# 001cat/pySurfInv

Hardware: AMD Instinct MI355X
Metric: layered-model dispersion forward solves/sec (20 periods) (higher is better)
Workload: dtype f32 (root search, Love group velocity) + f64 (Rayleigh eigenfunction state)

## Files before the change

pysurfinv_amd/csrc/surfdisp_kernels.hip:

```cpp
#include <hip/hip_runtime.h>
#include <stdint.h>
#include <type_traits>
#include <atomic>
#include "surfdisp_internal.h"

#define SD_HD __host__ __device__
#ifndef SD_CERT_STRIDE
#define SD_CERT_STRIDE 6
#endif

namespace sd {

constexpr float R0      = 6371.0f;
constexpr float PI_REF  = 3.1415927f;
constexpr float DC      = 0.01f;
constexpr float FACT    = 4.0f;
constexpr float ACCUR   = 1.e-8f;
constexpr float CLUSTER_DC = 1.0e-4f;

enum { F_VP = 0, F_VS, F_RHO, F_QS, F_DIF, F_QQQ, F_DFL, F_HSF, F_HSR, NF = 9 };

SD_HD __forceinline__ bool fin(float x) { return fabsf(x) <= 3.402823466e38f; }
SD_HD __forceinline__ float pwr_of(int kind) { return kind == 1 ? 5.0f : 2.2750f; }

// ... 1493 lines not shown
    const int mmf = (hk >> 16) & 0x3fff;
    const size_t fs = (size_t)A.Lmax * B;
    const float c = A.c[idx], T = A.per[k];
    struct Replay { int kk, nflat; float lnT; };
    const Replay r0{k, hk & 0xffff, logf(1.0f / T)};
    auto layer = [&](int i, Replay &r) -> LayerV {
        while (r.nflat <= i && r.kk > 0) {
            --r.kk;
            const int h = A.hist[(size_t)r.kk * B + b];
            r.nflat = (h < 0) ? n : (h & 0xffff);
            r.lnT = logf(1.0f / A.per[r.kk]);
        }
        return layer_derive(layer_load(A.mdl, fs, (size_t)i * B + b), r.lnT, i == r.nflat - 1);
    };
    const int last = mmf - 1;
    float v2 = 0.0f, v3 = 0.0f;
    bool exact = A.only_flagged != 0;
    if (!exact) {
        const RTrial t = ray_trial(c, T);
        int kk = k;
        int nflat = hk & 0xffff;
        float lnT = r0.lnT;
        RState s2{}, s3{};
        float phi = 0.0f, rho_prev = 0.0f;
        RLyr y{};
        float rho_i = 0.0f;
        for (int i = 0; i <= last; ++i) {
            while (nflat <= i && kk > 0) {
                --kk;
                const int h = A.hist[(size_t)kk * B + b];
                nflat = (h < 0) ? n : (h & 0xffff);
                lnT = logf(1.0f / A.per[kk]);
            }
            const LayerV v = layer_derive(layer_load(A.mdl, fs, (size_t)i * B + b), lnT, i == nflat - 1);
            rho_prev = rho_i;
            rho_i = v.rho;
            y.sv = v.b; y.d = v.d;
            y.ia2 = wk_ia2(v.a);
            y.ib2 = wk_ib2(v.b);
            y.rat = (i > 0) ? wk_rat(rho_prev, rho_i) : 0.0f;
            if (i == 0) {
                const float irho0 = wk_irho(rho_i);
                s2 = ray_start(t, 2, irho0);
                s3 = ray_start(t, 3, irho0);
                if (last >= 1) { ray_step<true>(s2, t, y, 2, phi); ray_step<true>(s3, t, y, 3, phi); }
            } else if (i < last) {
                ray_step<false>(s2, t, y, 2, phi);
                ray_step<false>(s3, t, y, 3, phi);
            }
        }
        const float rp = (last >= 1) ? rho_prev : 0.0f;
        float m2 = 0.0f, m3 = 0.0f;
        v2 = ray_close(s2, t, y, rho_i, rp, 2, &m2); v3 = ray_close(s3, t, y, rho_i, rp, 3, &m3);
        const float b2max = A.ovf ? 0.5f * __expf(0.25f * A.ovf[2 * (size_t)B + b]) : 0.0f;
        exact = (A.ell_ambig < 0.0f) ||
                ((A.ell_ambig > 0.0f) && (fabsf(v2) < A.ell_ambig * m2 || fabsf(v3) < A.ell_ambig * m3 || 2.0f * b2max > A.ell_gmax * c * c));
    }
    if (exact) {
        Replay r = r0;
        v2 = delta_rayleigh_ref_gen([&](int m) { const LayerV v = layer(m, r); return RefLyr{v.a, v.b, v.rho, v.d}; }, mmf, c, T, 2);
        r = r0;
        v3 = delta_rayleigh_ref_gen([&](int m) { const LayerV v = layer(m, r); return RefLyr{v.a, v.b, v.rho, v.d}; }, mmf, c, T, 3);
        if (A.amb_count) atomicAdd(A.amb_count + 1, 1);
    }
    A.ratio[idx] = 0.5f * v3 / v2;
}

struct Drop { int hs_layer; int nreg_hs; };

template <int KIND>
SD_HD __forceinline__ Drop drop_group(const float *__restrict__ mdl, size_t fs, int B, int b,
                                           int n, float lnT, float c, float T, int ndiv, bool water,
                                           float div)
{
    const float dmax = FACT * T * c;
    float sum = 0.0f;
    Drop r; r.hs_layer = n - 1; r.nreg_hs = 0;
    LayerRaw nraw = layer_load(mdl, fs, (size_t)b);
    for (int jl = 0; jl < n; ++jl) {
        const LayerRaw raw = nraw;
        if (jl + 1 < n) nraw = layer_load(mdl, fs, (size_t)(jl + 1) * B + b);
        const LayerV v = layer_derive(raw, lnT, jl == n - 1);
        if (!(c < v.b)) continue;
        if (jl == n - 1) break;
        const int nsub = (jl == 0 && water) ? 1 : ndiv;
        const float dsub = (ndiv > 1 && !(jl == 0 && water)) ? v.d / div : v.d;
        for (int s = 0; s < nsub; ++s) sum = sum + dsub;
        if (!(sum > dmax)) continue;
        const LayerV nx = layer_derive(nraw, lnT, jl + 1 == n - 1);
        bool lower, equal;
        if (KIND == 2) {
            lower = (nx.a < v.a) || (nx.a == v.a && nx.b < v.b);
            equal = (nx.a == v.a) && (nx.b == v.b);
        } else {
            lower = nx.b < v.b;
            equal = nx.b == v.b;
        }
        if (lower) { r.hs_layer = jl; r.nreg_hs = nsub - 1; break; }
        if (equal) continue;
        r.hs_layer = jl + 1; r.nreg_hs = 0; break;
    }
    return r;
}

struct KOut {
    float *b;
    size_t stride;
    ptrdiff_t off_a, off_r;
    int raw;
    SD_HD void put(int i, float vb, float va, float vr) const
    {
        float *q = b + (size_t)i * stride;
        *q = vb;
        if (off_a) *reinterpret_cast<float *>(reinterpret_cast<char *>(q) + off_a) = va;
        if (off_r) *reinterpret_cast<float *>(reinterpret_cast<char *>(q) + off_r) = vr;
    }
};
struct K3 { float b, a, r; };
struct Chain { float dbdb, dadb, dada, rfac; };
SD_HD __forceinline__ Chain chain_of(const LayerRaw &r, float lnT, bool is_halfspace, bool raw)
{
    if (raw) return Chain{1.0f, 0.0f, 1.0f, 1.0f};
    const float qsq = r.qs * lnT / PI_REF;
    const float qpq = qsq * 1.33333333f * (r.b_ref * r.b_ref) / (r.a_ref * r.a_ref);
    const float vfac = is_halfspace ? r.hsf : r.dif;
    Chain ch;
    ch.dbdb = (1.0f + qsq) * vfac;
    ch.dadb = 2.66666667f * qsq * (r.b_ref / r.a_ref) * vfac;
    ch.dada = (1.0f - qpq) * vfac;
    ch.rfac = is_halfspace ? r.hsr : r.qqq;
    return ch;
}
struct KC { float b1, b2, a, r; };
SD_HD __forceinline__ KC kern_coef(const LayerRaw &raw, const LayerV &v, float lnT, bool is_halfspace, float cw, bool rawc)
{
    const Chain ch = chain_of(raw, lnT, is_halfspace, rawc);
    const float rc2 = 2.0f * v.rho * cw;
    return KC{rc2 * v.b * ch.dbdb, rc2 * v.a * ch.dadb, rc2 * v.a * ch.dada, cw * ch.rfac / v.rho};
}
#ifndef SD_KERN_REAL
#define SD_KERN_REAL double
#endif
typedef SD_KERN_REAL KR;
SD_HD __forceinline__ K3 kern_layer_rayleigh(const KC &kc, float rho, float xlamb, float xmu, float wvno, float wvnosq,
                                             float omegsq, KR dmmr, KR dmmz, KR drsz, KR dzsr, KR smmz, KR smmr)
{
    const KR two = 2, k2 = wvnosq, tk = 2.0f * wvno;
    const KR dldl = -k2 * dmmr + tk * drsz - smmz;
    const KR dldm = -k2 * (two * dmmr + dmmz) - tk * dzsr - (two * smmz + smmr);
    const KR dldr = (KR)omegsq * (dmmr + dmmz);
    return K3{(float)((KR)kc.b1 * (dldm - two * dldl) + (KR)kc.b2 * dldl), (float)((KR)kc.a * dldl),
              (float)((KR)kc.r * ((KR)rho * dldr + (KR)xlamb * dldl + (KR)xmu * dldm))};
}

struct RCoef { float a12, a13, a21, a24, a31, a34, a42, a43, ddz; };

struct RInt {
    double i0, i1, i2;
};

struct M2x2 { double a, b, c, d; };
SD_HD __forceinline__ M2x2 mm(const M2x2 &x, const M2x2 &y)
{
#pragma clang fp contract(off)
    M2x2 r;
    r.a = fma(x.a, y.a, x.b * y.c); r.b = fma(x.a, y.b, x.b * y.d);
    r.c = fma(x.c, y.a, x.d * y.c); r.d = fma(x.c, y.b, x.d * y.d);
    return r;
}
SD_HD __forceinline__ M2x2 mm2(const M2x2 &x, const M2x2 &y, const M2x2 &u, const M2x2 &v)
{
#pragma clang fp contract(off)
    M2x2 r;
    r.a = fma(x.a, y.a, fma(x.b, y.c, fma(u.a, v.a, u.b * v.c))); r.b = fma(x.a, y.b, fma(x.b, y.d, fma(u.a, v.b, u.b * v.d)));
    r.c = fma(x.c, y.a, fma(x.d, y.c, fma(u.c, v.a, u.d * v.c))); r.d = fma(x.c, y.b, fma(x.d, y.d, fma(u.c, v.b, u.d * v.d)));
    return r;
}
SD_HD __forceinline__ M2x2 madd(const M2x2 &x, const M2x2 &y)
{
    M2x2 r; r.a = x.a + y.a; r.b = x.b + y.b; r.c = x.c + y.c; r.d = x.d + y.d; return r;
}
struct RProp { M2x2 p11, p12, p21, p22; };

SD_HD __forceinline__ RProp make_prop(const RCoef &q)
{
#pragma clang fp contract(off)
    const double wh = (double)(0.5f * q.ddz), w1 = (double)(1.0f * q.ddz);
    const double t6 = (double)((1.0f / 6.0f) * q.ddz), t3 = (double)((1.0f / 3.0f) * q.ddz);
    const double k1 = (t6 + t3) + (t3 + t6);
    const double k2 = (t3 * wh + t3 * wh) + t6 * w1;
    const double k3 = t3 * wh * wh + t6 * w1 * wh;
    const double k4 = t6 * w1 * wh * wh;
    const M2x2 m1 = {(double)q.a31, (double)q.a34, (double)q.a21, (double)q.a24};
    const M2x2 m2 = {(double)q.a13, (double)q.a12, (double)q.a43, (double)q.a42};
    RProp P;
    auto diag_block = [&](const M2x2 &nn) -> M2x2 {
        const double tr = nn.a + nn.d;
        const double det = fma(nn.a, nn.d, -(nn.b * nn.c));
        const double al = fma(k4, tr, k2), be = fma(-k4, det, 1.0);
        return M2x2{fma(al, nn.a, be), al * nn.b, al * nn.c, fma(al, nn.d, be)};
    };
    auto off_block = [&](const M2x2 &nn, const M2x2 &m) -> M2x2 {
        const M2x2 q = {fma(k3, nn.a, k1), k3 * nn.b, k3 * nn.c, fma(k3, nn.d, k1)};
        return mm(q, m);
    };
    {
        const M2x2 n1 = mm(m1, m2);
        P.p11 = diag_block(n1);
        P.p12 = off_block(n1, m1);
    }
    {
        const M2x2 n2 = mm(m2, m1);
        P.p22 = diag_block(n2);
        P.p21 = off_block(n2, m2);
    }
    return P;
}
struct RPow { double f0, f1, g0, g1; };
struct RBase { M2x2 m1, m2, n1, n2; double t, d; RPow p; };
SD_HD __forceinline__ RBase make_base(const RCoef &q)
{
#pragma clang fp contract(off)
    const double wh = (double)(0.5f * q.ddz), w1 = (double)(1.0f * q.ddz);
    const double t6 = (double)((1.0f / 6.0f) * q.ddz), t3 = (double)((1.0f / 3.0f) * q.ddz);
    const double k1 = (t6 + t3) + (t3 + t6);
    const double k2 = (t3 * wh + t3 * wh) + t6 * w1;
    const double k3 = t3 * wh * wh + t6 * w1 * wh;
    const double k4 = t6 * w1 * wh * wh;
    RBase r;
    r.m1 = M2x2{(double)q.a31, (double)q.a34, (double)q.a21, (double)q.a24};
    r.m2 = M2x2{(double)q.a13, (double)q.a12, (double)q.a43, (double)q.a42};
    r.n1 = mm(r.m1, r.m2);
    r.n2 = mm(r.m2, r.m1);
    r.t = r.n1.a + r.n1.d;
    r.d = fma(r.n1.a, r.n1.d, -(r.n1.b * r.n1.c));
    r.p = RPow{fma(-k4, r.d, 1.0), fma(k4, r.t, k2), k1, k3};
    return r;
}
SD_HD __forceinline__ RPow pow_mul(const RPow &x, const RPow &y, double t, double d)
{
#pragma clang fp contract(off)
    const double ff = x.f1 * y.f1, gg = x.g1 * y.g1, fg = fma(x.f1, y.g1, x.g1 * y.f1);
    const double a0 = fma(x.f0, y.f0, -d * ff), a1 = fma(x.f0, y.f1, fma(x.f1, y.f0, t * ff));
    const double b0 = fma(x.g0, y.g0, -d * gg), b1 = fma(x.g0, y.g1, fma(x.g1, y.g0, t * gg));
    RPow r;
    r.f0 = fma(-d, b1, a0);
    r.f1 = fma(t, b1, a1 + b0);
    r.g0 = fma(x.f0, y.g0, fma(x.g0, y.f0, -d * fg));
    r.g1 = fma(x.f0, y.g1, fma(x.f1, y.g0, fma(x.g0, y.f1, fma(x.g1, y.f0, t * fg))));
    return r;
}
SD_HD __forceinline__ RPow pow_sq(const RPow &x, double t, double d)
{
#pragma clang fp contract(off)
    const double ff = x.f1 * x.f1, gg = x.g1 * x.g1, fg = x.f1 * x.g1;
    const double a0 = fma(x.f0, x.f0, -d * ff), a1 = fma(2.0 * x.f0, x.f1, t * ff);
    const double b0 = fma(x.g0, x.g0, -d * gg), b1 = fma(2.0 * x.g0, x.g1, t * gg);
    RPow r;
    r.f0 = fma(-d, b1, a0);
    r.f1 = fma(t, b1, a1 + b0);
    r.g0 = 2.0 * fma(x.f0, x.g0, -d * fg);
    r.g1 = 2.0 * fma(x.f0, x.g1, fma(x.f1, x.g0, t * fg));
    return r;
}
SD_HD __forceinline__ RPow pow_sublayers(const RBase &L, int nreg)
{
    RPow q = pow_sq(pow_sq(L.p, L.t, L.d), L.t, L.d);
    RPow r = (nreg & 1) ? q : RPow{1.0, 0.0, 0.0, 0.0};
    for (int e = nreg >> 1; e > 0; e >>= 1) {
        q = pow_sq(q, L.t, L.d);
        if (e & 1) r = pow_mul(r, q, L.t, L.d);
    }
    return r;
}
SD_HD __forceinline__ RProp pow_expand(const RBase &L, const RPow &x)
{
#pragma clang fp contract(off)
    RProp P;
    P.p11 = M2x2{fma(x.f1, L.n1.a, x.f0), x.f1 * L.n1.b, x.f1 * L.n1.c, fma(x.f1, L.n1.d, x.f0)};
    P.p22 = M2x2{fma(x.f1, L.n2.a, x.f0), x.f1 * L.n2.b, x.f1 * L.n2.c, fma(x.f1, L.n2.d, x.f0)};
    P.p12 = mm(M2x2{fma(x.g1, L.n1.a, x.g0), x.g1 * L.n1.b, x.g1 * L.n1.c, fma(x.g1, L.n1.d, x.g0)}, L.m1);
    P.p21 = mm(M2x2{fma(x.g1, L.n2.a, x.g0), x.g1 * L.n2.b, x.g1 * L.n2.c, fma(x.g1, L.n2.d, x.g0)}, L.m2);
    return P;
}
SD_HD __forceinline__ RProp prop_sq(const RProp &P)
{
    RProp Q;
    Q.p11 = mm2(P.p11, P.p11, P.p12, P.p21);
    Q.p12 = mm2(P.p11, P.p12, P.p12, P.p22);
    Q.p21 = mm2(P.p21, P.p11, P.p22, P.p21);
    Q.p22 = mm2(P.p21, P.p12, P.p22, P.p22);
    return Q;
}
SD_HD __forceinline__ void prop_apply(const RProp &P, double v[4])
{
#pragma clang fp contract(off)
    const double ur = v[0], uz = v[1], tz = v[2], tr = v[3];
    v[0] = fma(P.p11.a, ur, fma(P.p11.b, tz, fma(P.p12.a, uz, P.p12.b * tr)));
    v[2] = fma(P.p11.c, ur, fma(P.p11.d, tz, fma(P.p12.c, uz, P.p12.d * tr)));
    v[1] = fma(P.p21.a, ur, fma(P.p21.b, tz, fma(P.p22.a, uz, P.p22.b * tr)));
    v[3] = fma(P.p21.c, ur, fma(P.p21.d, tz, fma(P.p22.c, uz, P.p22.d * tr)));
}

template <int MODE, bool KERN = false>
SD_HD __forceinline__ void rayleigh_sweep(const float *__restrict__ mdl, size_t fs, int B, int b,
                                               int n, float lnT, int ndiv, bool water, float div,
                                               const Drop dr, float wvno, float wvnosq, float omegsq,
                                               double y[4], double z[4], bool do_y,
                                               double xnorm, double bbn, RInt &acc,
                                               const KOut ko = KOut{nullptr, 1, 0, 0, 0}, float cw = 0.0f, K3 *hold = nullptr)
{
#pragma clang fp contract(off)
    LayerRaw nraw = layer_load(mdl, fs, (size_t)dr.hs_layer * B + b);
    for (int jl = dr.hs_layer; jl >= 0; --jl) {
        const LayerRaw raw = nraw;
        if (jl > 0) nraw = layer_load(mdl, fs, (size_t)(jl - 1) * B + b);
        const int nsub = (jl == 0 && water) ? 1 : ndiv;
        const int nreg = (jl == dr.hs_layer) ? dr.nreg_hs : nsub;
        if (nreg <= 0) continue;
        const LayerV v = layer_derive(raw, lnT, jl == n - 1);
        if (v.b <= 0.0f) {
            if (MODE == 2 && KERN && jl > 0) ko.put(jl, 0.0f, 0.0f, 0.0f);
            continue;
        }
        const float dsub = (ndiv > 1 && !(jl == 0 && water)) ? v.d / div : v.d;
        const float xmu = v.rho * v.b * v.b;
        const float xlamb = v.rho * (v.a * v.a - 2.0f * v.b * v.b);
        KC kc{};
        if (MODE == 2 && KERN) kc = kern_coef(raw, v, lnT, jl == n - 1, cw, ko.raw != 0);
        RCoef q;
        q.ddz = -dsub / (4.0f * 1.0f);
        q.a12 = 1.0f / (xlamb + 2.0f * xmu);
        q.a13 = wvno * xlamb * q.a12;
        q.a21 = -omegsq * v.rho;
        q.a24 = wvno; q.a31 = -wvno;
        q.a34 = 1.0f / xmu;
        q.a42 = -q.a13;
        q.a43 = q.a21 + 4.0f * wvnosq * xmu * (xlamb + xmu) * q.a12;
        if (MODE == 0) {
            const RBase L = make_base(q);
            const RProp Pm = pow_expand(L, pow_sublayers(L, nreg));
            if (do_y) prop_apply(Pm, y);
            prop_apply(Pm, z);
            continue;
        }
        const RProp P = make_prop(q);
        if (MODE == 1) {
            for (int s = 0; s < nreg; ++s) {
#pragma unroll
                for (int kk = 3; kk >= 0; --kk) {
                    if (do_y) prop_apply(P, y);
                    prop_apply(P, z);
                }
            }
            continue;
        }
        const bool two_vec = do_y;
        const float dz = dsub / 4.0f;
        const float l2m = xlamb + 2.0f * xmu;
        const float ixmu = q.a34, il2m = q.a12;
        float f_mr[5], f_mz[5], f_rz[5], f_zr[5];
        constexpr bool kern = KERN;
        KR k_mr = 0, k_mz = 0, k_rz = 0, k_zr = 0, k_sz = 0, k_sr = 0;
#ifdef SD_KERN_BOOLE_INCR
        float w_sz = 0.0f, w_sr = 0.0f, t_sz = 0.0f, t_sr = 0.0f;
#else
        float f_sz[5], f_sr[5];
#endif
        const double ibb = 1.0 / bbn;
        auto knot = [&](int kk) {
            float aur, auz, atz, atr;
            if (two_vec) {
                aur = (float)((xnorm * y[0] + z[0]) * ibb); auz = (float)((xnorm * y[1] + z[1]) * ibb);
                atz = (float)((xnorm * y[2] + z[2]) * ibb); atr = (float)((xnorm * y[3] + z[3]) * ibb);
            } else {
                aur = (float)z[0]; auz = (float)z[1]; atz = (float)z[2]; atr = (float)z[3];
            }
            const float durdz = atr * ixmu - wvno * auz;
            const float duzdz = (atz + wvno * xlamb * aur) * il2m;
            f_mr[kk] = aur * aur; f_mz[kk] = auz * auz;
            f_rz[kk] = aur * duzdz; f_zr[kk] = auz * durdz;
            if (kern) {
#ifdef SD_KERN_BOOLE_INCR
                t_sz = duzdz * duzdz; t_sr = durdz * durdz;
                const float wk = (kk == 2) ? 12.0f : ((kk & 1) ? 32.0f : 7.0f);
                w_sz = fmaf(wk, t_sz, w_sz); w_sr = fmaf(wk, t_sr, w_sr);
#else
                f_sz[kk] = duzdz * duzdz; f_sr[kk] = durdz * durdz;
#endif
            }
        };
        for (int s = 0; s < nreg; ++s) {
            if (s == 0) knot(4);
            else { f_mr[4] = f_mr[0]; f_mz[4] = f_mz[0]; f_rz[4] = f_rz[0]; f_zr[4] = f_zr[0];
#ifdef SD_KERN_BOOLE_INCR
                   if (kern) { w_sz = 7.0f * t_sz; w_sr = 7.0f * t_sr; }
#else
                   if (kern) { f_sz[4] = f_sz[0]; f_sr[4] = f_sr[0]; }
#endif
            }
#pragma unroll
            for (int kk = 3; kk >= 0; --kk) {
                if (two_vec) prop_apply(P, y);
                prop_apply(P, z);
                knot(kk);
            }
            const float hq = dz / 22.5f;
#define SD_BOOLE(v) (hq * (7.0f * (v[0] + v[4]) + 32.0f * (v[1] + v[3]) + 12.0f * v[2]))
            const float dmmr = SD_BOOLE(f_mr), dmmz = SD_BOOLE(f_mz);
            const float drsz = SD_BOOLE(f_rz), dzsr = SD_BOOLE(f_zr);
            if (kern) {
                k_mr += dmmr; k_mz += dmmz; k_rz += drsz; k_zr += dzsr;
#ifdef SD_KERN_BOOLE_INCR
                k_sz += hq * w_sz; k_sr += hq * w_sr;
#else
                k_sz += SD_BOOLE(f_sz); k_sr += SD_BOOLE(f_sr);
#endif
            }
#undef SD_BOOLE
            acc.i0 += (double)(v.rho * (dmmr + dmmz));
            acc.i1 += (double)(l2m * dmmr + xmu * dmmz);
            acc.i2 += (double)(xmu * dzsr - xlamb * drsz);
        }
        if (kern) {
            const K3 sh = kern_layer_rayleigh(kc, v.rho, xlamb, xmu, wvno, wvnosq, omegsq, k_mr, k_mz, k_rz, k_zr, k_sz, k_sr);
            if (jl == dr.hs_layer) *hold = sh;
            else ko.put(jl, sh.b, sh.a, sh.r);
        }
    }
}

#ifdef SD_COUNT_RESTARTS
__device__ unsigned long long sd_restart_count[2];
#endif

template <bool KERN = false>
SD_HD float group_rayleigh(const float *__restrict__ mdl, size_t fs, int B, int b, int n,
                                float T, float c, float ratio, double *dbg = nullptr,
                                const KOut ko = KOut{nullptr, 1, 0, 0, 0}, float *kscale = nullptr, int *khs = nullptr)
{
#pragma clang fp contract(off)
    const float lnT = logf(1.0f / T);
    int ndiv = 5;
    const int ivre = 99 / (n - 1);
    if (ndiv > ivre) ndiv = ivre;
    if (ndiv < 1) ndiv = 1;
    const float div = (float)ndiv;
    const LayerV top = layer_at(mdl, fs, (size_t)b, lnT, false);
    const bool water = (ndiv > 1) ? (top.b <= 0.1e-10f) : false;
    const bool wet = !(top.b > 0.0f);
    const Drop dr = drop_group<2>(mdl, fs, B, b, n, lnT, c, T, ndiv, water, div);
    const float wvno = 6.2831853072f / (c * T);
    const float wvnosq = wvno * wvno;
    const float omega = 6.2831853072f / T;
    const float omegsq = omega * omega;
    RInt acc; acc.i0 = 0.0; acc.i1 = 0.0; acc.i2 = 0.0;
    float tzz = 0.0f;
    const float cw = c / wvno;
    K3 hold{0.0f, 0.0f, 0.0f};
    if (KERN) { *kscale = 0.0f; *khs = dr.hs_layer; }
    float wat_a = 0.0f, wat_r = 0.0f;
    if (wet) {
        const float d1 = top.d;
        const float xl1 = top.rho * (top.a * top.a - 2.0f * top.b * top.b);
        const float ra = c / top.a;
        const float cr1 = ra * ra - 1.0f;
        const float mag = wvno * sqrtf(fabsf(cr1));
        if (mag <= 1.0e-35f) {
            acc.i0 = top.rho * d1;
        } else {
            float sin2ra, cosra, rab1, sinra_over;
            if (cr1 >= 0.0f) {
                sin2ra = sinf(2.0f * mag * d1) / (4.0f * mag);
                cosra = cosf(mag * d1);
                rab1 = mag * mag;
                sinra_over = sinf(mag * d1) / mag;
            } else {
                sin2ra = sinhf(2.0f * mag * d1) / (4.0f * mag);
                cosra = coshf(mag * d1);
                rab1 = -(mag * mag);
                sinra_over = sinhf(mag * d1) / mag;
            }
            const float cos2rm = 1.0f / (cosra * cosra);
            const float fac1 = (0.5f * d1 + sin2ra) * cos2rm;
            const float fac3 = wvno * (0.5f * d1 - sin2ra) * cos2rm;
            const float fac2 = wvno * fac3 / rab1;
            acc.i0 = top.rho * (fac1 + fac2);
            acc.i1 = xl1 * fac2;
            acc.i2 = xl1 * fac3;
            tzz = -top.rho * omegsq * sinra_over / cosra;
            if (KERN && !ko.raw) {
                const LayerRaw wraw = layer_load(mdl, fs, (size_t)b);
                const Chain ch = chain_of(wraw, lnT, false, false);
                const float dldl = -wvnosq * (ra * ra) * (ra * ra) * fac2;
                const float dldr = omegsq * (fac1 + fac2);
                wat_a = 2.0f * top.rho * top.a * cw * dldl * ch.dada;
                wat_r = cw * (dldr + top.a * top.a * dldl) * ch.rfac;
            }
        }
        if (KERN) ko.put(0, 0.0f, wat_a, wat_r);
    }
    const LayerV hsv = layer_at(mdl, fs, (size_t)dr.hs_layer * B + b, lnT, dr.hs_layer == n - 1);
    const float cova = c / hsv.a, covb = c / hsv.b;
    const float gam = 2.0f / (covb * covb);
    const float gamm1 = gam - 1.0f;
    const float ra = wvno * sqrtf(fabsf(cova * cova - 1.0f));
    const float rb = wvno * sqrtf(fabsf(covb * covb - 1.0f));
    const float det = wvnosq - ra * rb;
    const float h = hsv.rho * omegsq;
    const float brkt = -gamm1 * wvno + gam * ra * rb / wvno;
    const double y0[4] = {1.0, 0.0, (double)(-h * brkt / det), (double)(-h * ra / det)};
    double z0[4] = {0.0, 1.0, (double)(-h * rb / det), (double)(-h * brkt / det)};
    double y[4], z[4];
    double xnorm = 0.0, bbn = 1.0;
    auto fit = [&](auto step_tag) -> double {
        constexpr int STEP = decltype(step_tag)::value;
        for (int i = 0; i < 4; ++i) { y[i] = y0[i]; z[i] = z0[i]; }
        rayleigh_sweep<STEP>(mdl, fs, B, b, n, lnT, ndiv, water, div, dr, wvno, wvnosq, omegsq,
                             y, z, true, 0.0, 1.0, acc);
        const double yt0 = y[0], yt1 = y[1];
        double aa = z[0] - ratio * z[1];
        double bb = ratio * yt1 - yt0;
        if (fabs(bb) < 1.e-10) bb = copysign(1.e-10, bb);
        xnorm = aa / bb;
        bb = xnorm * yt1 + z[1];
        if (fabs(bb) < 1.e-10) bb = copysign(1.e-10, bb);
        bbn = bb;
        const float ampur = (float)((xnorm * yt0 + z[0]) / bb);
        const float xtest = fabsf(ampur / ratio - 1.0f);
#if defined(SD_COUNT_RESTARTS) && defined(__HIP_DEVICE_COMPILE__)
        if (STEP == 0) {
            const unsigned long long m = __ballot(xtest >= 0.00001f);
            if (m && (__lane_id() == __ffsll(__ballot(1)) - 1)) atomicAdd(&sd_restart_count[1], 1ull);
            if (xtest >= 0.00001f) atomicAdd(&sd_restart_count[0], 1ull);
        }
#endif
        if (xtest >= 0.00001f) {
            for (int i = 0; i < 4; ++i) z0[i] = z0[i] + xnorm * y0[i];
            if (STEP == 0) {
                for (int i = 0; i < 4; ++i) z[i] = z[i] + xnorm * y[i];
            } else {
                for (int i = 0; i < 4; ++i) z[i] = z0[i];
                rayleigh_sweep<STEP>(mdl, fs, B, b, n, lnT, ndiv, water, div, dr, wvno, wvnosq, omegsq,
                                     y, z, false, 0.0, 1.0, acc);
            }
            aa = z[0] - ratio * z[1];
            bb = ratio * yt1 - yt0;
            if (fabs(bb) < 1.e-10) bb = copysign(1.e-10, bb);
            xnorm = aa / bb;
            bb = xnorm * yt1 + z[1];
            if (fabs(bb) < 1.e-10) bb = copysign(1.e-10, bb);
            bbn = bb;
        }
        return fmax(fmax(fabs(yt0), fabs(yt1)), fmax(fabs(z[0]), fabs(z[1]))) / fabs(bbn);
    };
    const double z0_orig[4] = {z0[0], z0[1], z0[2], z0[3]};
    const double cancel = fit(std::integral_constant<int, 0>{});
    if (dbg) { for (int i = 0; i < 4; ++i) { dbg[i] = y[i]; dbg[4 + i] = z[i]; } dbg[12] = dr.hs_layer; dbg[13] = dr.nreg_hs; dbg[14] = ndiv; dbg[8] = xnorm; dbg[9] = bbn; }
    float aur, auz;
    const bool any_solid = (dr.hs_layer > (wet ? 1 : 0)) || (dr.nreg_hs > 0);
    (void)tzz;
    if (cancel <= 1.0e7) {
        for (int i = 0; i < 4; ++i) { z[i] = (xnorm * y0[i] + z0[i]) / bbn; y[i] = 0.0; }
        aur = (float)z[0]; auz = (float)z[1];
        rayleigh_sweep<2, KERN>(mdl, fs, B, b, n, lnT, ndiv, water, div, dr, wvno, wvnosq, omegsq,
                                y, z, false, xnorm, bbn, acc, ko, cw, &hold);
    } else {
        for (int i = 0; i < 4; ++i) z0[i] = z0_orig[i];
        (void)fit(std::integral_constant<int, 1>{});
        for (int i = 0; i < 4; ++i) { y[i] = y0[i]; z[i] = z0[i]; }
        aur = (float)((xnorm * y0[0] + z0[0]) / bbn);
        auz = (float)((xnorm * y0[1] + z0[1]) / bbn);
        rayleigh_sweep<2, KERN>(mdl, fs, B, b, n, lnT, ndiv, water, div, dr, wvno, wvnosq, omegsq,
                                y, z, true, xnorm, bbn, acc, ko, cw, &hold);
    }
    if (wet && !any_solid) { aur = ratio; auz = 1.0f; }
    {
        const float xmu = hsv.rho * hsv.b * hsv.b;
        const float xlamb = hsv.rho * (hsv.a * hsv.a - 2.0f * hsv.b * hsv.b);
        const float ap = -hsv.rho * (wvno * aur + rb * auz) / det;
        const float bp = -hsv.rho * (-ra * aur / wvno - auz) / det;
        const float a1 = -wvno * ap / hsv.rho;
        const float a2 = -wvno * rb * bp / hsv.rho;
        const float a3 = ra * ap / hsv.rho;
        const float a4 = wvnosq * bp / hsv.rho;
        if (rb == 0.0f) return hsv.b;
        const double dmmr = a1 * a1 / (2.0f * ra) + 2.0f * a1 * a2 / (ra + rb) + a2 * a2 / (2.0f * rb);
        const double dmmz = a3 * a3 / (2.0f * ra) + 2.0f * a3 * a4 / (ra + rb) + a4 * a4 / (2.0f * rb);
        const double drsz = -a1 * a3 / 2.0f - (a1 * a4 * rb + a2 * a3 * ra) / (ra + rb) - a2 * a4 / 2.0f;
        const double dzsr = -a1 * a3 / 2.0f - (a1 * a4 * ra + a2 * a3 * rb) / (ra + rb) - a2 * a4 / 2.0f;
        acc.i0 += hsv.rho * (dmmr + dmmz);
        acc.i1 += (xlamb + 2.0f * xmu) * dmmr + xmu * dmmz;
        acc.i2 += xmu * dzsr - xlamb * drsz;
        if (KERN) {
            const float smmz = ra * a3 * a3 / 2.0f + 2.0f * ra * rb * a3 * a4 / (ra + rb) + rb * a4 * a4 / 2.0f;
            const float smmr = ra * a1 * a1 / 2.0f + 2.0f * ra * rb * a1 * a2 / (ra + rb) + rb * a2 * a2 / 2.0f;
            const LayerRaw hraw = layer_load(mdl, fs, (size_t)dr.hs_layer * B + b);
            const K3 sh = kern_layer_rayleigh(kern_coef(hraw, hsv, lnT, dr.hs_layer == n - 1, cw, ko.raw != 0), hsv.rho, xlamb, xmu,
                                              wvno, wvnosq, omegsq, (KR)dmmr, (KR)dmmz, (KR)drsz, (KR)dzsr, (KR)smmz, (KR)smmr);
            ko.put(dr.hs_layer, hold.b + sh.b, hold.a + sh.a, hold.r + sh.r);
        }
    }
    if (dbg) { dbg[10] = acc.i0; dbg[11] = acc.i1; dbg[15] = acc.i2; }
    const float s0 = (float)acc.i0, s1 = (float)acc.i1, s2 = (float)acc.i2;
    if (KERN) *kscale = 1.0f / (-2.0f * (wvno * s1 + s2));
    return (wvno * s1 + s2) / (omega * s0);
}

template <bool KERN = false>
SD_HD float group_love(const float *__restrict__ mdl, size_t fs, int B, int b, int n,
                            float T, float c, const KOut ko = KOut{nullptr, 1, 0, 0, 0}, float *kscale = nullptr, int *khs = nullptr)
{
    const float lnT = logf(1.0f / T);
    int ndiv = 5;
    const int ivre = 999 / (n - 1);
    if (ndiv > ivre) ndiv = ivre;
    if (ndiv < 1) ndiv = 1;
    const float div = (float)ndiv;
    const LayerV top = layer_at(mdl, fs, (size_t)b, lnT, false);
    const bool water = (ndiv > 1) ? (top.b <= 0.1e-10f) : false;
    const Drop dr = drop_group<1>(mdl, fs, B, b, n, lnT, c, T, ndiv, water, div);
    const float wvno = 6.2831853f / (c * T);
    const LayerV hsv = layer_at(mdl, fs, (size_t)dr.hs_layer * B + b, lnT, dr.hs_layer == n - 1);
    constexpr bool kern = KERN;
    const float wvnosq = wvno * wvno;
    const float omega = 6.2831853f / T, omegsq = omega * omega;
    const float cw = c / wvno;
    auto kern_layer = [&](int jl, const LayerRaw &raw, const LayerV &v, float dm, float sm) -> K3 {
        const Chain ch = chain_of(raw, lnT, jl == n - 1, ko.raw != 0);
        const float dldm = -(wvnosq * dm + sm);
        const float dldr = omegsq * dm;
        return K3{2.0f * v.rho * v.b * cw * dldm * ch.dbdb, 0.0f, cw * (dldr + v.b * v.b * dldm) * ch.rfac};
    };
    if (kern) { *kscale = 0.0f; *khs = dr.hs_layer; }
    float ut0 = 1.0f;
    for (int attempt = 0; attempt < 16; ++attempt) {
        float ut = ut0;
        K3 hold{0.0f, 0.0f, 0.0f};
        const float covb = c / hsv.b;
        const float hh = hsv.rho * hsv.b * hsv.b;
        const float rbh = wvno * sqrtf(fabsf(covb * covb - 1.0f));
        float tq = -hh * rbh * ut0;
        const float dm0 = (rbh == 0.0f) ? 1.0e25f : 0.5f / rbh;
        float sumi0 = hsv.rho * dm0;
        float sumi1 = hh * dm0;
        bool overflow = false;
        LayerRaw nraw = layer_load(mdl, fs, (size_t)dr.hs_layer * B + b);
        if (kern && rbh > 0.0f) hold = kern_layer(dr.hs_layer, nraw, hsv, dm0, 0.5f * rbh);
        for (int jl = dr.hs_layer; jl >= 0 && !overflow; --jl) {
            const LayerRaw raw = nraw;
            if (jl > 0) nraw = layer_load(mdl, fs, (size_t)(jl - 1) * B + b);
            const int nsub = (jl == 0 && water) ? 1 : ndiv;
            const int nreg = (jl == dr.hs_layer) ? dr.nreg_hs : nsub;
            if (nreg <= 0) continue;
            const LayerV v = layer_derive(raw, lnT, jl == n - 1);
            if (v.b == 0.0f) {
                if (fabsf(ut) > 1.0e10f) overflow = true;
                if (kern && jl != dr.hs_layer) ko.put(jl, 0.0f, 0.0f, 0.0f);
                continue;
            }
            const float dsub = (ndiv > 1 && !(jl == 0 && water)) ? v.d / div : v.d;
            const float cv = c / v.b;
            const float rb = wvno * sqrtf(fabsf(cv * cv - 1.0f));
            const float h = v.rho * v.b * v.b;
            const float dz = dsub / 4.0f;
            float yk[4], zk[4], ck[4];
#pragma unroll
            for (int kk = 0; kk < 4; ++kk) {
                const float xkk = (float)(kk + 1);
                const float q = rb * dz * xkk;
                if (c < v.b) {
                    const float ep = expf(q), emq = 1.0f / ep;
                    yk[kk] = (ep - emq) / (2.0f * rb);
                    zk[kk] = rb * rb * yk[kk];
                    ck[kk] = (ep + emq) / 2.0f;
                } else if (c == v.b) {
                    yk[kk] = dz * xkk; zk[kk] = 0.0f; ck[kk] = 1.0f;
                } else {
                    float sn, cs; sincosf(q, &sn, &cs);
                    yk[kk] = sn / rb; zk[kk] = -rb * sn; ck[kk] = cs;
                }
            }
            float k_dm = 0.0f, k_sm = 0.0f;
            for (int s = 0; s < nreg; ++s) {
                if (fabsf(ut) > 1.0e10f) { overflow = true; break; }
                float dmm[5], smm[5];
                dmm[0] = ut * ut;
                if (kern) smm[0] = (tq / h) * (tq / h);
                float eut = ut, ett = tq;
#pragma unroll
                for (int kk = 0; kk < 4; ++kk) {
                    eut = ck[kk] * ut - yk[kk] * tq / h;
                    ett = -h * zk[kk] * ut + ck[kk] * tq;
                    dmm[kk + 1] = eut * eut;
                    if (kern) smm[kk + 1] = (ett * ett) / (h * h);
                }
                ut = eut; tq = ett;
                const float dm = (dz / 22.5f) * (7.0f * (dmm[0] + dmm[4]) + 32.0f * (dmm[1] + dmm[3]) + 12.0f * dmm[2]);
                sumi0 = sumi0 + v.rho * dm;
                sumi1 = sumi1 + h * dm;
                if (kern) {
                    k_dm += dm;
                    k_sm += (dz / 22.5f) * (7.0f * (smm[0] + smm[4]) + 32.0f * (smm[1] + smm[3]) + 12.0f * smm[2]);
                }
            }
            if (kern && !overflow) {
                const K3 sh = kern_layer(jl, raw, v, k_dm, k_sm);
                if (jl == dr.hs_layer) { hold.b += sh.b; hold.r += sh.r; }
                else ko.put(jl, sh.b, 0.0f, sh.r);
            }
        }
        if (overflow) { ut0 = ut0 / 1.0e5f; continue; }
        if (kern) {
            ko.put(dr.hs_layer, hold.b, 0.0f, hold.r);
            *kscale = 1.0f / (-2.0f * wvno * sumi1);
        }
        sumi0 = sumi0 / (ut * ut);
        sumi1 = sumi1 / (ut * ut);
        return sumi1 / (c * sumi0);
    }
    return 0.0f;
}

template <int KIND, bool KERN>
#ifndef SD_GROUP_WAVES
#define SD_GROUP_WAVES 3
#endif
#ifndef SD_KERN_WAVES
#define SD_KERN_WAVES 1
#endif
__global__ __launch_bounds__(256) __attribute__((amdgpu_waves_per_eu(KERN ? SD_KERN_WAVES : SD_GROUP_WAVES, 8)))
void surfdisp_group_kernel(GroupArgs A)
{
    const int B = A.B, P = A.P;
    size_t idx = (size_t)blockIdx.x * blockDim.x + threadIdx.x;
    int b, k;
    if (A.xcd_order) {
        const int g = A.xcd_order;
        const int x = blockIdx.x & 7, q = blockIdx.x >> 3;
        const int r = q % (g * P);
        k = r / g;
        b = (((q / (g * P)) * g + r % g) * 8 + x) * 256 + (int)threadIdx.x;
        if (b >= B) return;
        if (A.krev) k = P - 1 - k;
        idx = (size_t)k * B + b;
    } else {
        if (idx >= (size_t)B * P) return;
        b = (int)(idx % B); k = (int)(idx / B);
        if (A.krev) { k = P - 1 - k; idx = (size_t)k * B + b; }
    }
    const size_t o = idx;
    const int n = A.nl[b];
    KOut ko{nullptr, 1, 0, 0, 0};
    float *ra_ = nullptr, *rr_ = nullptr;
    if (KERN) {
        ko.raw = A.kraw;
        if (A.kscr) {
            const size_t arr = (size_t)A.Lmax * P * B;
            ko.stride = (size_t)P * B;
            ko.b = A.kscr + idx;
            ko.off_a = (KIND == 2 && A.ka) ? (ptrdiff_t)(arr * sizeof(float)) : 0;
            ko.off_r = A.kr ? (ptrdiff_t)(2 * arr * sizeof(float)) : 0;
        } else {
            const size_t ro = ((size_t)b * P + k) * A.Lmax;
            ko.stride = 1;
            ko.b = A.kb + ro;
            ra_ = A.ka ? A.ka + ro : nullptr;
            rr_ = A.kr ? A.kr + ro : nullptr;
            ko.off_a = (KIND == 2 && A.ka) ? (ptrdiff_t)(reinterpret_cast<const char *>(A.ka) - reinterpret_cast<const char *>(A.kb)) : 0;
            ko.off_r = A.kr ? (ptrdiff_t)(reinterpret_cast<const char *>(A.kr) - reinterpret_cast<const char *>(A.kb)) : 0;
        }
    }
    float kscale = 0.0f;
    int khs = -1;
    float ugr = 0.0f;
    if (n >= 2 && k < A.nsolved[b]) {
        const size_t fs = (size_t)A.Lmax * B;
        const float T = A.per[k];
        const float c = A.c[o];
        if (KIND == 2) ugr = group_rayleigh<KERN>(A.mdl, fs, B, b, n, T, c, A.ratio[(size_t)k * B + b],
                                                  A.dbg ? A.dbg + 16 * o : nullptr, ko, &kscale, &khs);
        else           ugr = group_love<KERN>(A.mdl, fs, B, b, n, T, c, ko, &kscale, &khs);
    }
    if (KERN) {
        if (!(fabsf(kscale) <= 3.0e38f)) kscale = 0.0f;
        if (A.kscr) { A.kscale[o] = kscale; A.khs[o] = (kscale != 0.0f) ? khs : -1; }
        else {
            const int top = (kscale != 0.0f) ? khs : -1;
            for (int i = 0; i < A.Lmax; ++i) {
                ko.b[i] = (i <= top) ? ko.b[i] * kscale : 0.0f;
                if (ra_) ra_[i] = (KIND == 2 && i <= top) ? ra_[i] * kscale : 0.0f;
                if (rr_) rr_[i] = (i <= top) ? rr_[i] * kscale : 0.0f;
            }
        }
    }
    A.u[o] = ugr;
}

__global__ __launch_bounds__(256) void surfdisp_finish_kernel(FinishArgs A)
{
    extern __shared__ float tile[];
    const int B = A.B, P = A.P, PS = P + 1;
    const int b0 = blockIdx.x * 64;
    const int nb = min(64, B - b0);
    if (A.nsolved && threadIdx.x < nb) {
        const int bb = b0 + threadIdx.x;
        const int ns = A.nsolved[bb];
        if (A.status) A.status[bb] = (A.nl[bb] < 2) ? SURFDISP_BADMODEL
                                     : (ns >= P ? SURFDISP_OK
                                     : (ns < 0 ? SURFDISP_NUMERIC : (ns == 0 ? SURFDISP_NOROOT : SURFDISP_PARTIAL)));
    }
    for (int pass = 0; pass < 3; ++pass) {
        const float *src = (pass == 0) ? A.ct : (pass == 1 ? A.ut : A.rt);
        float *dst = (pass == 0) ? A.c : (pass == 1 ? A.u : A.ratio);
        if (!src || !dst) continue;
        for (int i = threadIdx.x; i < 64 * P; i += 256) {
            const int k = i / 64, bl = i % 64;
            if (bl < nb) {
                float v = src[(size_t)k * B + b0 + bl];
                if (A.nsolved && k >= A.nsolved[b0 + bl]) v = 0.0f;
                if (pass == 2 && (k >= A.nsolved_all[b0 + bl] || A.nl[b0 + bl] < 2)) v = 0.0f;
                tile[bl * PS + k] = v;
            }
        }
        __syncthreads();
        for (int i = threadIdx.x; i < nb * P; i += 256) {
            const int bl = i / P, k = i % P;
            dst[(size_t)b0 * P + i] = tile[bl * PS + k];
        }
        __syncthreads();
    }
}

__global__ __launch_bounds__(256) void surfdisp_kern_transpose_kernel(KernTransposeArgs A)
{
    __shared__ float tile[64][65];
    const int B = A.B, P = A.P, Lmax = A.Lmax;
    float *__restrict__ out = (blockIdx.z == 0) ? A.kb : ((blockIdx.z == 1) ? A.ka : A.kr);
    if (!out) return;
    const float *__restrict__ scr = A.kscr + (size_t)blockIdx.z * Lmax * P * B;
    const bool zero_only = (blockIdx.z == 1) && (A.kind != 2);
    const int nbb = (B + 63) / 64;
    const int k = blockIdx.x / nbb, b0 = (blockIdx.x % nbb) * 64, i0 = blockIdx.y * 64;
    const size_t PB = (size_t)P * B;
    const int bl = threadIdx.x % 64;
    float sc = 0.0f; int hs = -1;
    if (b0 + bl < B && !zero_only) { sc = A.kscale[(size_t)k * B + b0 + bl]; hs = A.khs[(size_t)k * B + b0 + bl]; }
    for (int il = threadIdx.x / 64; il < 64; il += 4)
        tile[il][bl] = (i0 + il <= hs) ? scr[(size_t)(i0 + il) * PB + (size_t)k * B + b0 + bl] * sc : 0.0f;
    __syncthreads();
    for (int t = threadIdx.x; t < 64 * 64; t += 256) {
        const int bq = t / 64, il = t % 64;
        if (i0 + il < Lmax && b0 + bq < B) out[((size_t)(b0 + bq) * P + k) * Lmax + i0 + il] = tile[il][bq];
    }
}

#ifndef SD_SHIFT_WIDEN
#define SD_SHIFT_WIDEN 6
#endif
struct ShiftStack { const float *mdl; size_t fs; int B, b, n; float T, lnT; };
__device__ __forceinline__ LayerV shift_layer(const ShiftStack &q, int i)
{
    return layer_at(q.mdl, q.fs, (size_t)i * q.B + q.b, q.lnT, i == q.n - 1);
}
__device__ __forceinline__ int shift_drop(const ShiftStack &q, float c)
{
    const float dmax = FACT * c * q.T;
    int cnt = 0;
    float sum = 0.0f;
    for (int ii = 0; ii < q.n; ++ii) {
        const LayerV v = shift_layer(q, ii);
        sum = sum + ((c < v.b) ? v.d : 0.0f);
        cnt += (sum > dmax) ? 0 : 1;
    }
    const int mm = (cnt < q.n) ? cnt + 1 : q.n;
    return mm < 2 ? 2 : mm;
}
// ... 364 lines not shown
```

Before: 40.85 million.

## Adaptively coarsen Rayleigh sublayer steps using a local wavenumber bound

Adds a heuristic, fast_sublayers, that estimates each layer's local exponent (lam^2 * H^2) and picks fewer propagation sub-steps (up to 5) when the layer is thin relative to the wavelength. Sub-step thickness is enlarged to match. This cuts propagator applications and Boole quadrature knots in the eigenfunction sweep and the integral sweep. If the fit reports heavy cancellation after coarsening, it falls back to the original subdivision, which adds an occasional re-sweep and some risk to the accuracy of the energy integrals.

```diff
diff --git a/pysurfinv_amd/csrc/surfdisp_kernels.hip b/pysurfinv_amd/csrc/surfdisp_kernels.hip
--- a/pysurfinv_amd/csrc/surfdisp_kernels.hip
+++ b/pysurfinv_amd/csrc/surfdisp_kernels.hip
@@ -1819,13 +1819,33 @@
     v[3] = fma(P.p21.c, ur, fma(P.p21.d, tz, fma(P.p22.c, uz, P.p22.d * tr)));
 }
 
+#ifndef SD_GROUP_LAMH
+#define SD_GROUP_LAMH 0.05f
+#endif
+#ifndef SD_GROUP_OWN_CANCEL
+#define SD_GROUP_OWN_CANCEL 1.0e5
+#endif
+SD_HD __forceinline__ int fast_sublayers(const RCoef &q, float wvnosq, float dsub, int nreg)
+{
+    if (!(SD_GROUP_LAMH > 0.0f)) return nreg;
+    const float lam2 = fmaxf(fabsf(fmaf(q.a21, q.a12, wvnosq)), fabsf(fmaf(q.a21, q.a34, wvnosq)));
+    const float H = dsub * (float)nreg;
+    const float x = lam2 * H * H;
+    constexpr float t = 16.0f * SD_GROUP_LAMH * SD_GROUP_LAMH;
+    int m = 1;
+#pragma unroll
+    for (int i = 1; i < 5; ++i) m += (x > t * (float)(i * i)) ? 1 : 0;
+    return m < nreg ? m : nreg;
+}
+
 template <int MODE, bool KERN = false>
 SD_HD __forceinline__ void rayleigh_sweep(const float *__restrict__ mdl, size_t fs, int B, int b,
                                                int n, float lnT, int ndiv, bool water, float div,
                                                const Drop dr, float wvno, float wvnosq, float omegsq,
-                                               double y[4], double z[4], bool do_y,
+                                               double y[4], double z[4], bool do_y, bool own,
                                                double xnorm, double bbn, RInt &acc,
-                                               const KOut ko = KOut{nullptr, 1, 0, 0, 0}, float cw = 0.0f, K3 *hold = nullptr)
+                                               const KOut ko = KOut{nullptr, 1, 0, 0, 0}, float cw = 0.0f, K3 *hold = nullptr,
+                                               bool *shorter = nullptr)
 {
 #pragma clang fp contract(off)
     LayerRaw nraw = layer_load(mdl, fs, (size_t)dr.hs_layer * B + b);
@@ -1840,13 +1860,12 @@
             if (MODE == 2 && KERN && jl > 0) ko.put(jl, 0.0f, 0.0f, 0.0f);
             continue;
         }
-        const float dsub = (ndiv > 1 && !(jl == 0 && water)) ? v.d / div : v.d;
+        float dsub = (ndiv > 1 && !(jl == 0 && water)) ? v.d / div : v.d;
         const float xmu = v.rho * v.b * v.b;
         const float xlamb = v.rho * (v.a * v.a - 2.0f * v.b * v.b);
         KC kc{};
         if (MODE == 2 && KERN) kc = kern_coef(raw, v, lnT, jl == n - 1, cw, ko.raw != 0);
         RCoef q;
-        q.ddz = -dsub / (4.0f * 1.0f);
         q.a12 = 1.0f / (xlamb + 2.0f * xmu);
         q.a13 = wvno * xlamb * q.a12;
         q.a21 = -omegsq * v.rho;
@@ -1854,9 +1873,21 @@
         q.a34 = 1.0f / xmu;
         q.a42 = -q.a13;
         q.a43 = q.a21 + 4.0f * wvnosq * xmu * (xlamb + xmu) * q.a12;
+        int nstep = nreg;
+        if (MODE != 1 && own) {
+            nstep = fast_sublayers(q, wvnosq, dsub, nreg);
+            if (nstep < nreg) {
+                dsub = (dsub * (float)nreg) / (float)nstep;
+                if (shorter) *shorter = true;
+            }
+        }
+#ifdef SD_SPLIT_PROBE
+        if (MODE == 2 && !do_y) SD_SPLIT_PROBE(nreg, nstep);
+#endif
+        q.ddz = -dsub / (4.0f * 1.0f);
         if (MODE == 0) {
             const RBase L = make_base(q);
-            const RProp Pm = pow_expand(L, pow_sublayers(L, nreg));
+            const RProp Pm = pow_expand(L, pow_sublayers(L, nstep));
             if (do_y) prop_apply(Pm, y);
             prop_apply(Pm, z);
             continue;
@@ -1907,7 +1938,7 @@
 #endif
             }
         };
-        for (int s = 0; s < nreg; ++s) {
+        for (int s = 0; s < nstep; ++s) {
             if (s == 0) knot(4);
             else { f_mr[4] = f_mr[0]; f_mz[4] = f_mz[0]; f_rz[4] = f_rz[0]; f_zr[4] = f_zr[0];
 #ifdef SD_KERN_BOOLE_INCR
@@ -2030,11 +2061,12 @@
     double z0[4] = {0.0, 1.0, (double)(-h * rb / det), (double)(-h * brkt / det)};
     double y[4], z[4];
     double xnorm = 0.0, bbn = 1.0;
-    auto fit = [&](auto step_tag) -> double {
+    bool shorter = false;
+    auto fit = [&](auto step_tag, bool own) -> double {
         constexpr int STEP = decltype(step_tag)::value;
         for (int i = 0; i < 4; ++i) { y[i] = y0[i]; z[i] = z0[i]; }
         rayleigh_sweep<STEP>(mdl, fs, B, b, n, lnT, ndiv, water, div, dr, wvno, wvnosq, omegsq,
-                             y, z, true, 0.0, 1.0, acc);
+                             y, z, true, own, 0.0, 1.0, acc, KOut{nullptr, 1, 0, 0, 0}, 0.0f, nullptr, &shorter);
         const double yt0 = y[0], yt1 = y[1];
         double aa = z[0] - ratio * z[1];
         double bb = ratio * yt1 - yt0;
@@ -2059,7 +2091,7 @@
             } else {
                 for (int i = 0; i < 4; ++i) z[i] = z0[i];
                 rayleigh_sweep<STEP>(mdl, fs, B, b, n, lnT, ndiv, water, div, dr, wvno, wvnosq, omegsq,
-                                     y, z, false, 0.0, 1.0, acc);
+                                     y, z, false, false, 0.0, 1.0, acc);
             }
             aa = z[0] - ratio * z[1];
             bb = ratio * yt1 - yt0;
@@ -2072,7 +2104,14 @@
         return fmax(fmax(fabs(yt0), fabs(yt1)), fmax(fabs(z[0]), fabs(z[1]))) / fabs(bbn);
     };
     const double z0_orig[4] = {z0[0], z0[1], z0[2], z0[3]};
-    const double cancel = fit(std::integral_constant<int, 0>{});
+    bool own = SD_GROUP_LAMH > 0.0f;
+    double cancel;
+    for (;;) {
+        cancel = fit(std::integral_constant<int, 0>{}, own);
+        if (!own || !shorter || !(cancel > SD_GROUP_OWN_CANCEL) || cancel > 1.0e7) break;
+        own = false;
+        for (int i = 0; i < 4; ++i) z0[i] = z0_orig[i];
+    }
     if (dbg) { for (int i = 0; i < 4; ++i) { dbg[i] = y[i]; dbg[4 + i] = z[i]; } dbg[12] = dr.hs_layer; dbg[13] = dr.nreg_hs; dbg[14] = ndiv; dbg[8] = xnorm; dbg[9] = bbn; }
     float aur, auz;
     const bool any_solid = (dr.hs_layer > (wet ? 1 : 0)) || (dr.nreg_hs > 0);
@@ -2081,15 +2120,15 @@
         for (int i = 0; i < 4; ++i) { z[i] = (xnorm * y0[i] + z0[i]) / bbn; y[i] = 0.0; }
         aur = (float)z[0]; auz = (float)z[1];
         rayleigh_sweep<2, KERN>(mdl, fs, B, b, n, lnT, ndiv, water, div, dr, wvno, wvnosq, omegsq,
-                                y, z, false, xnorm, bbn, acc, ko, cw, &hold);
+                                y, z, false, own, xnorm, bbn, acc, ko, cw, &hold);
     } else {
         for (int i = 0; i < 4; ++i) z0[i] = z0_orig[i];
-        (void)fit(std::integral_constant<int, 1>{});
+        (void)fit(std::integral_constant<int, 1>{}, false);
         for (int i = 0; i < 4; ++i) { y[i] = y0[i]; z[i] = z0[i]; }
         aur = (float)((xnorm * y0[0] + z0[0]) / bbn);
         auz = (float)((xnorm * y0[1] + z0[1]) / bbn);
         rayleigh_sweep<2, KERN>(mdl, fs, B, b, n, lnT, ndiv, water, div, dr, wvno, wvnosq, omegsq,
-                                y, z, true, xnorm, bbn, acc, ko, cw, &hold);
+                                y, z, true, false, xnorm, bbn, acc, ko, cw, &hold);
     }
     if (wet && !any_solid) { aur = ratio; auz = 1.0f; }
     {
```

Result: faster. 41.76 million (median of 6 runs) (+2.2%).
